# Kelicious/faster_rcnn

Hardware: AMD Instinct MI355X
Metric: images/sec end-to-end (RPN+det) ResNet-50 600x1000 (higher is better)
Workload: dtype f32

## Files before the change

faster_rcnn_amd/_lib.py:

```python
import ctypes
import os
from ctypes import c_char_p, c_double, c_int, c_size_t, c_void_p

HERE = os.path.dirname(os.path.abspath(__file__))
LIB_PATH = os.environ.get("FRCNN_LIB_PATH") or os.path.join(HERE, "libfrcnn_hip.so")


class FrcnnError(RuntimeError):
    pass


ABI_VERSION = 110
P = c_void_p
I = c_int
SIGNATURES = {
    "frcnn_last_error": (c_char_p, []),
    "frcnn_version": (I, []),
    "frcnn_device_count": (I, []),
    "frcnn_preprocess_u8": (I, [P, c_size_t, P, P, P]),
    "frcnn_resize_cubic_taps": (I, [I, I, P]),
    "frcnn_resize_cubic_u8": (I, [P, I, I, P, P, I, I, I, P, P]),
    "frcnn_anchors_image": (I, [I, I, P, I, I, P, P]),
    "frcnn_anchors_conv": (I, [I, I, P, I, P, P]),
    "frcnn_cross_ious_f32": (I, [P, I, P, I, P, P]),
# ... 58 lines not shown
    "frcnn_conv2d_fwd_ws_amax": (I, [P, P, P, P, P, P, P, P, P, P, c_size_t, P]),
    "frcnn_pack_conv_weights_dgrad": (I, [P, P, I, I, I, I, P, P]),
    "frcnn_conv2d_wgrad_workspace_bytes": (c_size_t, [P]),
    "frcnn_conv2d_wgrad": (I, [P, P, P, P, P, P, P, c_size_t, P]),
    "frcnn_conv2d_wgrad_batch_workspace_bytes": (c_size_t, [P, I]),
    "frcnn_conv2d_wgrad_batch": (I, [P, I, P, c_size_t, P]),
    "frcnn_refresh_packed": (I, [P, I, P]),
    "frcnn_colsum_batch": (I, [P, I, P]),
    "frcnn_pool2d_fwd": (I, [P, I, I, I, I, I, I, I, P, P]),
    "frcnn_pool2d_fwd_planes": (I, [P, I, I, I, I, I, I, I, P, P]),
    "frcnn_avgpool_pos_major": (I, [P, I, I, I, P, P]),
    "frcnn_softmax_rows": (I, [P, I, I, I, P, I, P]),
    "frcnn_dense_heads_split": (I, [P, I, I, I, I, P, P, P]),
    "frcnn_loss_rpn_cls": (I, [P, P, I, I, P, P, P]),
    "frcnn_loss_rpn_reg": (I, [P, P, I, I, P, P, P]),
    "frcnn_loss_workspace_bytes": (ctypes.c_size_t, []),
    "frcnn_loss_rpn_cls_ws": (I, [P, P, I, I, P, P, P, P]),
    "frcnn_loss_rpn_reg_ws": (I, [P, P, I, I, P, P, P, P]),
    "frcnn_loss_det_cls": (I, [P, P, I, I, P, P, I, P]),
    "frcnn_loss_det_reg": (I, [P, P, I, I, P, P, I, P]),
    "frcnn_relu_bwd_inplace": (I, [P, P, c_size_t, P]),
    "frcnn_avgpool_bwd_masked": (I, [P, P, I, I, I, P, P]),
    "frcnn_maxpool_bwd": (I, [P, P, P, I, I, I, I, I, P, P]),
    "frcnn_sgd_momentum": (I, [P, P, P, c_size_t, ctypes.c_float, ctypes.c_float, ctypes.c_float, ctypes.c_float, P]),
    "frcnn_adam": (I, [P, P, P, P, c_size_t, ctypes.c_float, ctypes.c_float, ctypes.c_float, ctypes.c_float, I, ctypes.c_float, ctypes.c_float, P]),
    "frcnn_sumsq_workspace_bytes": (c_size_t, []),
    "frcnn_sumsq": (I, [P, c_size_t, P, P, c_size_t, P]),
    "frcnn_fold_bias": (I, [P, P, P, P, I, P]),
    "frcnn_stem_bf16_packed_elems": (I, []),
    "frcnn_pack_stem_weights_bf16": (I, [P, P, P]),
    "frcnn_stem_bf16_fwd": (I, [P, I, I, I, P, P, P, P, P]),
    "frcnn_conv_packed_k_bf16": (I, [I, I, I]),
    "frcnn_pack_conv_weights_bf16": (I, [P, I, I, I, I, P, P]),
    "frcnn_conv2d_fwd_bf16": (I, [P, P, P, P, P, P, P, I, P]),
    "frcnn_conv2d_workspace_bytes_bf16": (c_size_t, [P]),
    "frcnn_conv2d_fwd_bf16_ws": (I, [P, P, P, P, P, P, P, I, P, c_size_t, P]),
    "frcnn_conv2d_fwd_bf16_masked": (I, [P, P, P, P, P, P, P, P, I, P, c_size_t, P]),
    "frcnn_refresh_packed_bf16": (I, [P, I, P]),
    "frcnn_conv2d_wgrad_bf16": (I, [P, P, P, P, P, P, P, c_size_t, P]),
    "frcnn_cast_bf16_to_f32": (I, [P, c_size_t, P, P]),
    "frcnn_relu_bwd_inplace_bf16": (I, [P, P, c_size_t, P]),
    "frcnn_avgpool_bwd_masked_bf16": (I, [P, P, I, I, I, P, P]),
    "frcnn_roi_crop_resize_bwd_bf16": (I, [P, I, I, I, P, I, I, P, P]),
    "frcnn_cast_f32_to_bf16": (I, [P, c_size_t, P, P]),
    "frcnn_avgpool_bf16_to_f32": (I, [P, I, I, I, P, P]),
    "frcnn_avgpool_bf16_to_f32_ex": (I, [P, I, I, I, I, P, P]),
    "frcnn_roi_crop_resize_fwd_bf16": (I, [P, I, I, I, P, I, I, P, P]),
    "frcnn_roi_crop_resize_fwd_bf16_ex": (I, [P, I, I, I, P, I, I, P, I, I, P, P]),
    "frcnn_roi_crop_resize_fwd_bf16_batch": (I, [P, I, I, I, I, P, I, I, P, I, I, P, P]),
    "frcnn_detections": (I, [P, P, I, P, P, I, I, c_double, c_double, c_double, c_double, P, P, P, P, P, P]),
    "frcnn_detections_dyn": (I, [P, P, I, I, P, P, I, I, c_double, c_double, P, P, P, P, P, P, P]),
    "frcnn_annotate_u8": (I, [P, I, I, P, P, P, P, I, P, P, I, I, P, P]),
    "frcnn_vgg_conv1_bf16_packed_elems": (I, []),
    "frcnn_pack_vgg_conv1_weights_bf16": (I, [P, P, P]),
    "frcnn_vgg_conv1_bf16_fwd": (I, [P, I, I, I, P, P, P, P]),
    "frcnn_pool2d_fwd_bf16": (I, [P, I, I, I, I, I, I, P, P]),
}

VGG_CANVAS_VERSION = 1
EXT_SIGNATURES = {
    "frcnn_vgg_canvas_version": (I, []),
    "frcnn_pool2d_fwd_extents": (I, [P, I, I, I, I, P, P, P]),
    "frcnn_pool2d_fwd_bf16_extents": (I, [P, I, I, I, I, P, P, P]),
    "frcnn_vgg_conv1_bf16_fwd_extents": (I, [P, I, I, I, P, P, P, P, P]),
}

ROI_RES_VERSION = 1
ROI_TAP_BYTES = 32
ROI_RES_SIGNATURES = {
    "frcnn_roi_res_version": (I, []),
    "frcnn_roi_tap_table": (I, [I, I, I, P, I, I, I, I, I, P, P]),
    "frcnn_conv2d_roi_res_available": (I, [P, I, I]),
    "frcnn_conv2d_fwd_h3_roi_res": (I, [P, P, P, P, P, P, P, P, P, P, P, P, ctypes.c_float, ctypes.c_float, P]),
}


POOL_EPILOGUE_VERSION = 1
POOL_EPILOGUE_SIGNATURES = {
    "frcnn_pool_epilogue_version": (I, []),
    "frcnn_conv2d_pool_available": (I, [P, I, I, I]),
    "frcnn_conv2d_fwd_h3_pool": (I, [P, P, P, P, P, P, P, P, P, P, I, P, P, P, P]),
}


class RoiRes(ctypes.Structure):
    _fields_ = [("map", c_void_p), ("taps", c_void_p), ("fill", c_void_p), ("map_rows", ctypes.c_int32), ("reserved", ctypes.c_int32)]


PNG_VERSION = 1
PNG_SIGNATURES = {
    "frcnn_png_version": (I, []),
    "frcnn_png_band_rows": (I, []),
    "frcnn_png_bound": (c_size_t, [I, I]),
    "frcnn_png_workspace_bytes": (c_size_t, [I, I]),
    "frcnn_png_encode_u8": (I, [P, I, I, I, P, c_size_t, P, P, P]),
}

PNG_HUFF_VERSION = 1
PNG_HUFF_SIGNATURES = {
    "frcnn_png_huff_version": (I, []),
    "frcnn_png_huff_band_rows": (I, []),
    "frcnn_png_huff_bound": (c_size_t, [I, I]),
    "frcnn_png_huff_workspace_bytes": (c_size_t, [I, I]),
    "frcnn_png_huff_encode_u8": (I, [P, I, I, I, P, c_size_t, P, P, P]),
}

JPEG_VERSION = 1
JPEG_SIGNATURES = {
    "frcnn_jpeg_version": (I, []),
    "frcnn_jpeg_restart_mcus": (I, []),
    "frcnn_jpeg_header_bytes": (c_size_t, []),
    "frcnn_jpeg_bound": (c_size_t, [I, I]),
    "frcnn_jpeg_workspace_bytes": (c_size_t, [I, I]),
    "frcnn_jpeg_encode_u8": (I, [P, I, I, I, I, P, c_size_t, P, P, P]),
}

JPEG_OPT_VERSION = 1
JPEG_OPT_SIGNATURES = {
    "frcnn_jpeg_opt_version": (I, []),
    "frcnn_jpeg_opt_restart_mcus": (I, [I]),
    "frcnn_jpeg_opt_bound": (c_size_t, [I, I, I]),
    "frcnn_jpeg_opt_workspace_bytes": (c_size_t, [I, I, I, I]),
    "frcnn_jpeg_opt_encode_u8": (I, [P, I, I, I, I, I, I, P, c_size_t, P, P, P]),
    "frcnn_jpeg_opt_build_tables": (I, [P, P, P]),
}
JPEG_OPT_SUBSAMPLINGS = (444, 420)
JPEG_OPT_HUFFMANS = {"standard": 0, "optimized": 1}


class JpegOptTable(ctypes.Structure):
    _fields_ = [("bits", ctypes.c_uint8 * 16), ("huffval", ctypes.c_uint8 * 256), ("count", ctypes.c_uint32)]


JPEG_DEC_VERSION = 1
JPEG_DEC_SIGNATURES = {
    "frcnn_jpeg_dec_version": (I, []),
    "frcnn_jpeg_dec_plan": (I, [P, c_size_t, P]),
    "frcnn_jpeg_dec_workspace_bytes": (c_size_t, [P]),
    "frcnn_jpeg_decode_u8": (I, [P, P, I, P, c_size_t, P, P, P]),
}
JPEG_DEC_BATCH_VERSION = 1
JPEG_DEC_BATCH_MAX = 64
JPEG_DEC_BATCH_SIGNATURES = {
    "frcnn_jpeg_dec_batch_version": (I, []),
    "frcnn_jpeg_dec_batch_layout": (c_size_t, [P, I, P]),
    "frcnn_jpeg_decode_batch_u8": (I, [P, P, I, P, c_size_t, I, P, c_size_t, P, P, c_size_t, P]),
}
E_UNSUPPORTED = -4
JPEG_DEC_BLOCKS, JPEG_DEC_ZIGZAG, JPEG_DEC_CODE, JPEG_DEC_TABLE = 1, 2, 4, 8


PNG_DEC_VERSION = 1
PNG_DEC_BATCH_MAX = 64
PNG_DEC_WINDOW_BYTES = 8192
PNG_DEC_MAX_STREAM = 1 << 24
PNG_DEC_SIGNATURES = {
    "frcnn_png_dec_version": (I, []),
    "frcnn_png_dec_plan": (I, [P, c_size_t, P]),
    "frcnn_png_dec_spans": (I, [P, c_size_t, P, P, c_size_t]),
    "frcnn_png_dec_workspace_bytes": (c_size_t, [P]),
    "frcnn_png_dec_batch_layout": (c_size_t, [P, I, P]),
    "frcnn_png_decode_batch_u8": (I, [P, P, I, P, c_size_t, I, P, c_size_t, P, P, c_size_t, P]),
}
PNG_DEC_CODE, PNG_DEC_BLOCK, PNG_DEC_OVERSUBSCRIBED, PNG_DEC_DISTANCE, PNG_DEC_OVERRUN, PNG_DEC_UNDERRUN, PNG_DEC_ADLER, PNG_DEC_FILTER = \
    1, 2, 4, 8, 16, 32, 64, 128

# ... 154 lines not shown
    "frcnn_track_trails_update": (I, [P, I, P, ctypes.c_longlong, I, I, P, P, I, I, I, I, P, P]),
    "frcnn_track_trails_draw_u8": (I, [P, I, I, P, I, I, I, P]),
}
TRACK_TRAILS = ((2, 64, 16), (1, 9, 3), 4095)

TRACK_LOOKBACK_VERSION = 1
TRACK_LOOKBACK_SIGNATURES = {
    "frcnn_track_lookback_version": (I, []),
    "frcnn_track_lookback_state_bytes": (c_size_t, [I, I, I, I, I, I]),
    "frcnn_track_lookback": (I, [P, P, ctypes.c_longlong, P, ctypes.c_longlong, I, P, I, I, I, I, I, I, I, I, P, ctypes.c_longlong, P,
                                 ctypes.c_longlong, P, P]),
}
TRACK_LOOKBACK = (1, 16, 8)
TRACK_LOOKBACK_MAX_BACK = 128
TRACK_LOOKBACK_HEADER = 32

TRACK_BACKTRACK_VERSION = 1
TRACK_BACKTRACK_SIGNATURES = {
    "frcnn_track_backtrack_version": (I, []),
    "frcnn_track_backtrack": (I, [P, P, ctypes.c_longlong, P, ctypes.c_longlong, I, P, I, I, I, I, I, I, I, I, I, P, ctypes.c_longlong, P,
                                  ctypes.c_longlong, P, P]),
}


class ConvDesc(ctypes.Structure):
    _fields_ = [(k, ctypes.c_int32) for k in (
        "n", "h", "w", "cin", "cout", "kh", "kw", "stride", "pad_top", "pad_left", "ho", "wo",
        "act", "ldy", "ldres", "tile", "layout")]


class PackJob(ctypes.Structure):
    _fields_ = [(k, c_void_p) for k in ("w_hwio", "packed", "packed_dgrad", "bias", "scale", "shift_const", "shift")] + \
               [(k, ctypes.c_int32) for k in ("kh", "kw", "cin", "cout")]


class WgradJob(ctypes.Structure):
    _fields_ = [("d", ConvDesc)] + [(k, c_void_p) for k in ("x", "g", "scale", "dw")] + [(k, ctypes.c_int32) for k in ("in_bf16", "reserved")]


class X6Job(ctypes.Structure):
    _fields_ = [("w_packed", c_void_p), ("planes_bf16", c_void_p), ("rows", ctypes.c_int32), ("kpad", ctypes.c_int32)]


H3_UNDER, H3_SATURATED, H3_NONFINITE = 1, 2, 4


class H3Planes(ctypes.Structure):
    _fields_ = [("planes", c_void_p), ("exponent", c_void_p), ("status", c_void_p)]


class ColsumJob(ctypes.Structure):
    _fields_ = [(k, c_void_p) for k in ("g", "scale", "out")] + [(k, ctypes.c_int32) for k in ("m", "cout", "g_is_bf16", "reserved")]


_lib = None


def load():
    global _lib
    if _lib is not None:
        return _lib
    if not os.path.exists(LIB_PATH):
        raise FrcnnError(
            f"{LIB_PATH} is missing: build it with `python -m faster_rcnn_amd.build` "
            "(hipcc --offload-arch=gfx950).  There is no CPU fallback.")
    import torch
    lib = ctypes.CDLL(LIB_PATH)
    for name, (res, args) in SIGNATURES.items():
        fn = getattr(lib, name)
        fn.restype = res
        fn.argtypes = args
    for name, (res, args) in EXT_SIGNATURES.items():
        fn = getattr(lib, name)
        fn.restype = res
        fn.argtypes = args
    for name, (res, args) in ROI_RES_SIGNATURES.items():
        fn = getattr(lib, name)
        fn.restype = res
        fn.argtypes = args
    for name, (res, args) in POOL_EPILOGUE_SIGNATURES.items():
        fn = getattr(lib, name)
        fn.restype = res
        fn.argtypes = args
    for name, (res, args) in PNG_SIGNATURES.items():
        fn = getattr(lib, name)
        fn.restype = res
        fn.argtypes = args
    for name, (res, args) in PNG_HUFF_SIGNATURES.items():
        fn = getattr(lib, name)
        fn.restype = res
        fn.argtypes = args
    for name, (res, args) in JPEG_SIGNATURES.items():
        fn = getattr(lib, name)
        fn.restype = res
        fn.argtypes = args
    for name, (res, args) in JPEG_OPT_SIGNATURES.items():
        fn = getattr(lib, name)
        fn.restype = res
        fn.argtypes = args
    for name, (res, args) in JPEG_DEC_SIGNATURES.items():
        fn = getattr(lib, name)
        fn.restype = res
        fn.argtypes = args
    for name, (res, args) in JPEG_DEC_BATCH_SIGNATURES.items():
        fn = getattr(lib, name)
        fn.restype = res
        fn.argtypes = args
    for name, (res, args) in PNG_DEC_SIGNATURES.items():
        fn = getattr(lib, name)
        fn.restype = res
        fn.argtypes = args
    for name, (res, args) in PNG_DEC_FULL_SIGNATURES.items():
        fn = getattr(lib, name)
        fn.restype = res
        fn.argtypes = args
    for name, (res, args) in JPEG_DEC_FULL_SIGNATURES.items():
        fn = getattr(lib, name)
        fn.restype = res
        fn.argtypes = args
    for name, (res, args) in Y4M_SIGNATURES.items():
        fn = getattr(lib, name)
        fn.restype = res
        fn.argtypes = args
    for name, (res, args) in REDACT_SIGNATURES.items():
        fn = getattr(lib, name)
        fn.restype = res
        fn.argtypes = args
    for name, (res, args) in TRACK_SIGNATURES.items():
        fn = getattr(lib, name)
        fn.restype = res
        fn.argtypes = args
    if lib.frcnn_track_version() != TRACK_VERSION:
        raise FrcnnError(f"{LIB_PATH} speaks revision {lib.frcnn_track_version()} of the tracking extension, this binding "
                         f"{TRACK_VERSION} (include/ext/frcnn_hip_track.h): rebuild with `python -m faster_rcnn_amd.build`")
    for name, (res, args) in TRACK_MOTION_SIGNATURES.items():
        fn = getattr(lib, name)
        fn.restype = res
        fn.argtypes = args
    if lib.frcnn_track_motion_version() != TRACK_MOTION_VERSION:
        raise FrcnnError(f"{LIB_PATH} speaks revision {lib.frcnn_track_motion_version()} of the tracker's motion extension, this binding "
                         f"{TRACK_MOTION_VERSION} (include/ext/frcnn_hip_track_motion.h): rebuild with `python -m faster_rcnn_amd.build`")
    for name, (res, args) in TRACK_LOOKBACK_SIGNATURES.items():
        fn = getattr(lib, name)
        fn.restype = res
        fn.argtypes = args
    if lib.frcnn_track_lookback_version() != TRACK_LOOKBACK_VERSION:
        raise FrcnnError(f"{LIB_PATH} speaks revision {lib.frcnn_track_lookback_version()} of the tracker's look-back extension, this binding "
                         f"{TRACK_LOOKBACK_VERSION} (include/ext/frcnn_hip_track_lookback.h): rebuild with `python -m faster_rcnn_amd.build`")
    for name, (res, args) in TRACK_BACKTRACK_SIGNATURES.items():
        fn = getattr(lib, name, None)
        if fn is None:
            raise FrcnnError(f"{LIB_PATH} has no {name} (include/ext/frcnn_hip_track_backtrack.h): rebuild with `python -m faster_rcnn_amd.build`")
        fn.restype = res
        fn.argtypes = args
    if lib.frcnn_track_backtrack_version() != TRACK_BACKTRACK_VERSION:
        raise FrcnnError(f"{LIB_PATH} speaks revision {lib.frcnn_track_backtrack_version()} of the tracker's back-track extension, this binding "
                         f"{TRACK_BACKTRACK_VERSION} (include/ext/frcnn_hip_track_backtrack.h): rebuild with `python -m faster_rcnn_amd.build`")
    for name, (res, args) in TRACK_INTERVAL_SIGNATURES.items():
        fn = getattr(lib, name)
        fn.restype = res
        fn.argtypes = args
    if lib.frcnn_track_interval_version() != TRACK_INTERVAL_VERSION:
        raise FrcnnError(f"{LIB_PATH} speaks revision {lib.frcnn_track_interval_version()} of the tracker's interval extension, this binding "
                         f"{TRACK_INTERVAL_VERSION} (include/ext/frcnn_hip_track_interval.h): rebuild with `python -m faster_rcnn_amd.build`")
    for name, (res, args) in TRACK_CUT_SIGNATURES.items():
        fn = getattr(lib, name, None)
# ... 76 lines not shown
```

faster_rcnn_amd/csrc/stem_h3.hip:

```cpp
#include "conv_f32_common.h"

namespace frcnn {

typedef _Float16 sf16x8 __attribute__((ext_vector_type(8)));

constexpr int SH_PH = 4, SH_PW = 16;
constexpr int SH_CH = 2 * SH_PH + 1, SH_CW = 2 * SH_PW + 1;
constexpr int SH_CM = SH_CH * SH_CW;
constexpr int SH_MT = (SH_CM + 31) / 32;
constexpr int SH_IH = 2 * SH_CH + 5, SH_IW = 2 * SH_CW + 5;
constexpr int SH_ROW = 216;
constexpr int SH_PROWS = SH_IH + 2;
constexpr int SH_K = 176, SH_WLD = 184;
constexpr int SH_CLD = 68;
constexpr int SH_NT = 512;
constexpr size_t SH_PATCH = (size_t)SH_PROWS * SH_ROW * 2, SH_FILT = (size_t)64 * SH_WLD * 2;
constexpr size_t SH_LDS = 2 * SH_PATCH + 2 * SH_FILT + (size_t)SH_CM * SH_CLD * 4;
constexpr int SH_HEADER = 16;

__host__ __device__ __forceinline__ int sh_exponent(float amax) {
    unsigned b;
    __builtin_memcpy(&b, &amax, 4);
    const int e = 141 - (int)((b >> 23) & 0xffu);
    return e > 100 ? 100 : (e < -100 ? -100 : e);
}
__host__ __device__ __forceinline__ float sh_pow2(int e) {
    const unsigned b = (unsigned)(e + 127) << 23;
    float f;
    __builtin_memcpy(&f, &b, 4);
    return f;
}

__global__ void __launch_bounds__(SH_NT) k_stem_h3(const float* __restrict__ x, const float* __restrict__ x_amax, const char* __restrict__ wp,
                                                   const float* __restrict__ scale, const float* __restrict__ shift, int H, int W, int Hp, int Wp,
                                                   float* __restrict__ out, float* __restrict__ y_amax) {
    extern __shared__ __attribute__((aligned(16))) char sh_smem[];
    _Float16* patch = reinterpret_cast<_Float16*>(sh_smem);
    _Float16* wl = reinterpret_cast<_Float16*>(sh_smem + 2 * SH_PATCH);
    float* ct = reinterpret_cast<float*>(sh_smem + 2 * SH_PATCH + 2 * SH_FILT);
    const int tid = threadIdx.x, lane = tid & 63, wave = tid >> 6, li = lane & 31, lh = lane >> 5;
    const int px0 = blockIdx.x * SH_PW, py0 = blockIdx.y * SH_PH, img = blockIdx.z;
    const int Ho = (H + 1) / 2, Wo = (W + 1) / 2;
    const int pad_t = max((Ho - 1) * 2 + 7 - H, 0) / 2, pad_l = max((Wo - 1) * 2 + 7 - W, 0) / 2;
    const int iy0 = 4 * py0 - pad_t, ix0 = 4 * px0 - pad_l;
    const float* xi = x + (size_t)img * H * W * 3;

    constexpr int NP = (SH_PROWS * SH_ROW + SH_NT - 1) / SH_NT;
    float pv[NP];
#pragma unroll
    for (int q = 0; q < NP; ++q) {
        const int idx = tid + q * SH_NT;
        const int row = idx / SH_ROW, col = idx - row * SH_ROW;
        const int gy = iy0 + row, gx = ix0 + col / 3;
        const bool ok = idx < SH_PROWS * SH_ROW && row < SH_IH && col < SH_IW * 3 && (unsigned)gy < (unsigned)H && (unsigned)gx < (unsigned)W;
        pv[q] = ok ? xi[(size_t)gy * W * 3 + (ix0 * 3 + col)] : 0.0f;
    }
    h3_fp16_saturate();
    const float x_max = amax_read(x_amax);
    const int eA = sh_exponent(x_max);
    const int eB = sh_exponent(*reinterpret_cast<const float*>(wp));
    const float sA = sh_pow2(eA);
    h3_check_record(x_amax, x_max);
    unsigned seen = 0u;
#pragma unroll
    for (int q = 0; q < NP; ++q) {
        const int idx = tid + q * SH_NT;
        if (idx < SH_PROWS * SH_ROW) {
            const float xs = pv[q] * sA;
            const _Float16 hi = (_Float16)xs;
            h3_see(seen, hi);
            patch[idx] = hi;
            patch[SH_PROWS * SH_ROW + idx] = (_Float16)((xs - (float)hi) * 2048.0f);
        }
    }
    h3_report(x_amax, seen);
    const _Float16* wsrc = reinterpret_cast<const _Float16*>(wp + SH_HEADER);
    for (int idx = tid; idx < 2 * 64 * (SH_K / 8); idx += SH_NT) {
        const int pl = idx / (64 * (SH_K / 8)), r = idx - pl * (64 * (SH_K / 8)), n = r / (SH_K / 8), c8 = r - n * (SH_K / 8);
        *reinterpret_cast<i32x4*>(wl + pl * 64 * SH_WLD + n * SH_WLD + c8 * 8) = *reinterpret_cast<const i32x4*>(wsrc + pl * 64 * SH_K + n * SH_K + c8 * 8);
    }
    __syncthreads();

    const float unscale_a = sh_pow2(-eA), unscale_b = sh_pow2(-eB);
    for (int u = wave; u < 2 * SH_MT; u += SH_NT / 64) {
        const int mt = u >> 1, ct_col = (u & 1) * 32;
        const int m = mt * 32 + li, mm = m < SH_CM ? m : 0;
        const int cy = mm / SH_CW, cx = mm - cy * SH_CW;
        const _Float16* arow = patch + (2 * cy) * SH_ROW + 6 * cx;
        const _Float16* brow = wl + (ct_col + li) * SH_WLD + lh * 8;
        f32x16 acc0, acc1;
#pragma unroll
        for (int e = 0; e < 16; ++e) { acc0[e] = 0.0f; acc1[e] = 0.0f; }
#pragma unroll
        for (int kt = 0; kt < SH_K / 16; ++kt) {
            const int g = 2 * kt + lh, r = g / 3, j0 = (g - 3 * r) * 8;
            const unsigned* ah = reinterpret_cast<const unsigned*>(arow + r * SH_ROW + j0);
            const unsigned* al = ah + SH_PROWS * SH_ROW / 2;
            const i32x4 avh = {(int)ah[0], (int)ah[1], (int)ah[2], (int)ah[3]}, avl = {(int)al[0], (int)al[1], (int)al[2], (int)al[3]};
            const sf16x8 fah = __builtin_bit_cast(sf16x8, avh), fal = __builtin_bit_cast(sf16x8, avl);
            const sf16x8 fbh = *reinterpret_cast<const sf16x8*>(brow + kt * 16);
            const sf16x8 fbl = *reinterpret_cast<const sf16x8*>(brow + 64 * SH_WLD + kt * 16);
            acc1 = __builtin_amdgcn_mfma_f32_32x32x16_f16(fal, fbh, acc1, 0, 0, 0);
            acc1 = __builtin_amdgcn_mfma_f32_32x32x16_f16(fah, fbl, acc1, 0, 0, 0);
            acc0 = __builtin_amdgcn_mfma_f32_32x32x16_f16(fah, fbh, acc0, 0, 0, 0);
        }
        const float sc = scale[ct_col + li], sh = shift[ct_col + li];
#pragma unroll
        for (int e = 0; e < 16; ++e) {
            const int row = mt * 32 + (e & 3) + 8 * (e >> 2) + 4 * lh;
            if (row < SH_CM) {
                const float conv = ((acc0[e] + acc1[e] * (1.0f / 2048.0f)) * unscale_a) * unscale_b;
                ct[row * SH_CLD + ct_col + li] = fmaxf(conv * sc + sh, 0.0f);
            }
        }
    }
    __syncthreads();

    float vmax = 0.0f;
    for (int item = tid; item < SH_PH * SH_PW * 16; item += SH_NT) {
        const int pix = item >> 4, c4 = item & 15;
        const int ppy = pix / SH_PW, ppx = pix - ppy * SH_PW;
        const int py = py0 + ppy, px = px0 + ppx;
        if (py < Hp && px < Wp) {
            f32x4 best = {0.0f, 0.0f, 0.0f, 0.0f};
#pragma unroll
            for (int dy = 0; dy < 3; ++dy)
#pragma unroll
                for (int dx = 0; dx < 3; ++dx) {
                    const f32x4 v = *reinterpret_cast<const f32x4*>(ct + ((2 * ppy + dy) * SH_CW + 2 * ppx + dx) * SH_CLD + c4 * 4);
#pragma unroll
                    for (int q = 0; q < 4; ++q) best[q] = fmaxf(best[q], v[q]);
                }
            *reinterpret_cast<f32x4*>(out + (((size_t)img * Hp + py) * Wp + px) * 64 + c4 * 4) = best;
            vmax = fmaxf(fmaxf(vmax, fmaxf(best[0], best[1])), fmaxf(best[2], best[3]));
        }
    }
    if (y_amax) amax_publish(y_amax, vmax);
}

__global__ void k_stem_h3_wmax(const float* w, unsigned* header) {
    float v = 0.0f;
    for (int i = blockIdx.x * blockDim.x + threadIdx.x; i < 7 * 7 * 3 * 64; i += gridDim.x * blockDim.x) v = fmaxf(v, fabsf(w[i]));
    v = wave_max(v);
    if ((threadIdx.x & 63) == 0 && v > 0.0f) atomicMax(header, __float_as_uint(v));
}

__global__ void k_pack_stem_h3(const float* w, char* packed) {
    const float s = sh_pow2(sh_exponent(*reinterpret_cast<const float*>(packed)));
    _Float16* out = reinterpret_cast<_Float16*>(packed + SH_HEADER);
    for (int i = blockIdx.x * blockDim.x + threadIdx.x; i < 64 * SH_K; i += gridDim.x * blockDim.x) {
        const int n = i / SH_K, k = i - n * SH_K, r = k / 24, j = k - r * 24, sx = j / 3, c = j - sx * 3;
        const float v = (r < 7 && j < 21) ? w[((r * 7 + sx) * 3 + c) * 64 + n] * s : 0.0f;
        const _Float16 hi = (_Float16)v;
        out[i] = hi;
        out[64 * SH_K + i] = (_Float16)((v - (float)hi) * 2048.0f);
    }
}

__global__ void k_stem_h3_zero_header(unsigned* header) { if (threadIdx.x < SH_HEADER / 4) header[threadIdx.x] = 0u; }

}

using namespace frcnn;

extern "C" {

size_t frcnn_stem_h3_packed_bytes(void) { return (size_t)SH_HEADER + (size_t)2 * 64 * SH_K * 2; }

int frcnn_pack_stem_weights_h3(const float* w_hwio, void* packed, void* stream) {
    if (!w_hwio || !packed) return fail(FRCNN_E_ARG, "pack_stem_weights_h3: null pointer");
    if (reinterpret_cast<uintptr_t>(packed) & 15) return fail(FRCNN_E_ARG, "pack_stem_weights_h3: 16-byte aligned buffer required");
    hipStream_t s = as_stream(stream);
    k_stem_h3_zero_header<<<1, 64, 0, s>>>(reinterpret_cast<unsigned*>(packed));
    k_stem_h3_wmax<<<37, 256, 0, s>>>(w_hwio, reinterpret_cast<unsigned*>(packed));
    k_pack_stem_h3<<<44, 256, 0, s>>>(w_hwio, reinterpret_cast<char*>(packed));
    return check_launch("pack_stem_weights_h3");
}

int frcnn_stem_h3_fwd(const float* x, const float* x_amax, int n, int h, int w, const void* w_packed, const float* scale, const float* shift,
                      float* out, float* y_amax, void* stream) {
    if (!x || !x_amax || !w_packed || !scale || !shift || !out) return fail(FRCNN_E_ARG, "stem_h3_fwd: null pointer (the image's magnitude record is required)");
    if (n <= 0 || h < 7 || w < 7) return fail(FRCNN_E_ARG, "stem_h3_fwd: bad shape");
    const int ho = (h + 1) / 2, wo = (w + 1) / 2, hp = (ho - 3) / 2 + 1, wp = (wo - 3) / 2 + 1;
    if (hp <= 0 || wp <= 0) return fail(FRCNN_E_ARG, "stem_h3_fwd: image too small for the 3x3 pool");
    if ((reinterpret_cast<uintptr_t>(w_packed) | reinterpret_cast<uintptr_t>(out)) & 15) return fail(FRCNN_E_ARG, "stem_h3_fwd: 16-byte aligned tensors");
    static std::atomic<uint64_t> lds_seen{0};
    if (int e = raise_lds_once(lds_seen, (const void*)k_stem_h3, SH_LDS, "stem_h3_fwd")) return e;
    const dim3 grid((wp + SH_PW - 1) / SH_PW, (hp + SH_PH - 1) / SH_PH, n);
    if (grid.y > 65535 || grid.z > 65535) return fail(FRCNN_E_ARG, "stem_h3_fwd: image too large");
    k_stem_h3<<<grid, SH_NT, SH_LDS, as_stream(stream)>>>(x, x_amax, reinterpret_cast<const char*>(w_packed), scale, shift, h, w, hp, wp, out, y_amax);
    return check_launch("stem_h3_fwd");
}

}
```

faster_rcnn_amd/ops.py:

```python
import ctypes
import dataclasses
import os

import numpy as np
import torch

from . import _lib
from . import y4m as _y4m

NMS_MAX_BOXES = 12288


_GPU_SEEN = False


def _require_gpu():
    global _GPU_SEEN
    if not _GPU_SEEN:
        if not torch.cuda.is_available():
            raise _lib.FrcnnError("no HIP device visible: the faster_rcnn_amd ops need an MI355X (no CPU fallback)")
        _GPU_SEEN = True


_RAW_STREAM = getattr(torch._C, "_cuda_getCurrentRawStream", None)
# ... 2168 lines not shown
    _lib.call("frcnn_cast_f32_to_bf16", _p(x.contiguous()), x.numel(), _p(out), _stream())
    return out


def avgpool_bf16(x, k, layout=0):
    _require_gpu()
    n, c = (x.shape[2] if layout else x.shape[0]), x.shape[3]
    out = torch.empty((n, c), dtype=torch.float32, device="cuda")
    _lib.call("frcnn_avgpool_bf16_to_f32_ex", _p(x.contiguous()), n, k, c, layout, _p(out), _stream())
    return out


def roi_crop_resize_bf16(feat, rois, pool, fill=None, relu=False, layout=0):
    _require_gpu()
    feat = feat.reshape(feat.shape[-3], feat.shape[-2], feat.shape[-1]).contiguous()
    rows, cols, C = feat.shape
    rois = rois.reshape(-1, 4).to(torch.float32).contiguous()
    n = rois.shape[0]
    out = torch.empty((pool, pool, n, C) if layout else (n, pool, pool, C), dtype=torch.bfloat16, device="cuda")
    _lib.call("frcnn_roi_crop_resize_fwd_bf16_ex", _p(feat), rows, cols, C, _p(rois), n, pool, _p(fill), 1 if relu else 0, layout, _p(out), _stream())
    return out


def roi_crop_resize_bf16_batch(feat, rois, n_per_img, pool, fill=None, relu=False, layout=0):
    _require_gpu()
    assert feat.dtype == torch.bfloat16 and feat.dim() == 4 and feat.is_contiguous()
    B, rows, cols, C = feat.shape
    rois = rois.reshape(-1, 4).to(torch.float32).contiguous()
    n = rois.shape[0]
    assert n == B * n_per_img
    out = torch.empty((pool, pool, n, C) if layout else (n, pool, pool, C), dtype=torch.bfloat16, device="cuda")
    _lib.call("frcnn_roi_crop_resize_fwd_bf16_batch", _p(feat), B, rows, cols, C, _p(rois), n_per_img, pool, _p(fill), 1 if relu else 0, layout, _p(out), _stream())
    return out


class PackedStemBf16:

    def __init__(self, w_hwio, scale, shift):
        _require_gpu()
        w = _dev(w_hwio, torch.float32)
        assert tuple(w.shape) == (7, 7, 3, 64), "the fused stem is conv1 of the ResNets: 7x7x3 -> 64"
        self.w = torch.empty(_lib.load().frcnn_stem_bf16_packed_elems(), dtype=torch.bfloat16, device="cuda")
        _lib.call("frcnn_pack_stem_weights_bf16", _p(w), _p(self.w), _stream())
        self.scale, self.shift = _dev(scale, torch.float32), _dev(shift, torch.float32)
        torch.cuda.current_stream().synchronize()


def stem_bf16(x, ps):
    _require_gpu()
    assert x.dtype == torch.float32 and x.is_contiguous() and x.dim() == 4 and x.shape[-1] == 3
    n, h, w, _ = x.shape
    ho, wo = (h + 1) // 2, (w + 1) // 2
    out = torch.empty((n, (ho - 3) // 2 + 1, (wo - 3) // 2 + 1, 64), dtype=torch.bfloat16, device="cuda")
    _lib.call("frcnn_stem_bf16_fwd", _p(x), n, h, w, _p(ps.w), _p(ps.scale), _p(ps.shift), _p(out), _stream())
    return out


class PackedStemH3:

    def __init__(self, w_hwio, scale, shift):
        _require_gpu()
        w = _dev(w_hwio, torch.float32)
        assert tuple(w.shape) == (7, 7, 3, 64), "the fused stem is conv1 of the ResNets: 7x7x3 -> 64"
        self.w = torch.empty(_lib.load().frcnn_stem_h3_packed_bytes(), dtype=torch.uint8, device="cuda")
        _lib.call("frcnn_pack_stem_weights_h3", _p(w), _p(self.w), _stream())
        self.scale, self.shift = _dev(scale, torch.float32), _dev(shift, torch.float32)
        torch.cuda.current_stream().synchronize()


def stem_h3(x, ps):
    _require_gpu()
    assert x.dtype == torch.float32 and x.is_contiguous() and x.dim() == 4 and x.shape[-1] == 3
    n, h, w, _ = x.shape
    ho, wo = (h + 1) // 2, (w + 1) // 2
    out = torch.empty((n, (ho - 3) // 2 + 1, (wo - 3) // 2 + 1, 64), dtype=torch.float32, device="cuda")
    ya, xa = _amax_new(), amax_of(x)
    args = (_p(x), _p(xa), n, h, w, _p(ps.w), _p(ps.scale), _p(ps.shift), _p(out), _p(ya))
    _lib.call("frcnn_stem_h3_fwd", *args, _stream())
    out._amax = ya
    _record_launch(lambda: "k_stem_h3", (n * ho * wo, 64, 147, 2), "frcnn_stem_h3_fwd", args, (x, ps, out, ya, xa))
    return out


class PackedVggConv1Bf16:

    def __init__(self, w_hwio, bias):
        _require_gpu()
        w = _dev(w_hwio, torch.float32)
        assert tuple(w.shape) == (3, 3, 3, 64), "the conv1 kernel is block1_conv1 of VGG16: 3x3x3 -> 64"
        self.w = torch.empty(_lib.load().frcnn_vgg_conv1_bf16_packed_elems(), dtype=torch.bfloat16, device="cuda")
        _lib.call("frcnn_pack_vgg_conv1_weights_bf16", _p(w), _p(self.w), _stream())
        self.bias = _dev(bias, torch.float32)
        torch.cuda.current_stream().synchronize()


def vgg_conv1_bf16(x, packed):
    _require_gpu()
    assert x.dtype == torch.float32 and x.is_contiguous() and x.dim() == 4 and x.shape[-1] == 3
    n, h, w, _ = x.shape
    out = torch.empty((n, h, w, 64), dtype=torch.bfloat16, device="cuda")
    args = (_p(x), n, h, w, _p(packed.w), _p(packed.bias), _p(out))
    _lib.call("frcnn_vgg_conv1_bf16_fwd", *args, _stream())
    _record_launch(lambda: "k_vgg_conv1_bf16", (n * h * w, 64, 27, 1), "frcnn_vgg_conv1_bf16_fwd", args, (x, packed, out))
    return out


def pool2d_bf16(x, k, stride):
    _require_gpu()
    assert x.dtype == torch.bfloat16 and x.is_contiguous() and x.dim() == 4
    n, h, w, c = x.shape
    out = torch.empty((n, valid_out(h, k, stride), valid_out(w, k, stride), c), dtype=torch.bfloat16, device="cuda")
    args = (_p(x), n, h, w, c, k, stride, _p(out))
    _lib.call("frcnn_pool2d_fwd_bf16", *args, _stream())
    _record_launch(lambda: "k_pool2_bf16", (out.numel() // c, c, k * k, 1), "frcnn_pool2d_fwd_bf16", args, (x, out))
    return out


def vgg_conv1_bf16_extents(x, packed, true_hw):
    _require_gpu()
    assert x.dtype == torch.float32 and x.is_contiguous() and x.dim() == 4 and x.shape[-1] == 3
    assert true_hw.dtype == torch.int32 and true_hw.is_cuda and true_hw.numel() >= 2 * x.shape[0]
    n, h, w, _ = x.shape
    out = torch.empty((n, h, w, 64), dtype=torch.bfloat16, device="cuda")
    args = (_p(x), n, h, w, _p(packed.w), _p(packed.bias), _p(true_hw), _p(out))
    _lib.call("frcnn_vgg_conv1_bf16_fwd_extents", *args, _stream())
    _record_launch(lambda: "k_vgg_conv1_bf16", (n * h * w, 64, 27, 1), "frcnn_vgg_conv1_bf16_fwd_extents", args, (x, packed, out, true_hw))
    return out


def pool2d_bf16_extents(x, true_hw):
    _require_gpu()
    assert x.dtype == torch.bfloat16 and x.is_contiguous() and x.dim() == 4
    assert true_hw.dtype == torch.int32 and true_hw.is_cuda and true_hw.numel() >= 2 * x.shape[0]
    n, h, w, c = (int(v) for v in x.shape)
    out = torch.empty((n, h // 2, w // 2, c), dtype=torch.bfloat16, device="cuda")
    args = (_p(x), n, h, w, c, _p(true_hw), _p(out))
    _lib.call("frcnn_pool2d_fwd_bf16_extents", *args, _stream())
    _record_launch(lambda: "k_pool2_extents", (out.numel() // c, c, 4, 1), "frcnn_pool2d_fwd_bf16_extents", args, (x, out, true_hw))
    return out
```

Baseline: 560.9.

## Add persistent stem kernel with register-held filters and double-buffered patch prefetch

Adds a persistent form of the fused stem conv+BN+ReLU+maxpool kernel. A grid of at most one workgroup per compute unit walks the patches in a strided loop. Each wave keeps its filter fragments in registers instead of reloading them from LDS per patch. The next patch's global loads are issued before the MFMA work on the current patch, and the patch buffer is double-buffered in LDS. This is meant to amortise filter loading and block launch overhead and to hide input-load latency, at the cost of higher register pressure and only one 512-thread workgroup per CU. The persistent form is the default and can be turned off with an environment variable.

```diff
diff --git a/faster_rcnn_amd/_lib.py b/faster_rcnn_amd/_lib.py
--- a/faster_rcnn_amd/_lib.py
+++ b/faster_rcnn_amd/_lib.py
@@ -164,6 +164,15 @@
     "frcnn_conv2d_fwd_h3_pool": (I, [P, P, P, P, P, P, P, P, P, P, I, P, P, P, P]),
 }
 
+STEM_H3_PERSISTENT_VERSION = 1
+STEM_H3_FORM_PATCH, STEM_H3_FORM_PERSISTENT = 0, 1
+STEM_H3_PERSISTENT_SIGNATURES = {
+    "frcnn_stem_h3_persistent_version": (I, []),
+    "frcnn_stem_h3_default_form": (I, []),
+    "frcnn_stem_h3_workgroups": (I, [I, I, I, I, I]),
+    "frcnn_stem_h3_fwd_form": (I, [P, P, I, I, I, P, P, P, P, P, I, I, P]),
+}
+
 
 class RoiRes(ctypes.Structure):
     _fields_ = [("map", c_void_p), ("taps", c_void_p), ("fill", c_void_p), ("map_rows", ctypes.c_int32), ("reserved", ctypes.c_int32)]
@@ -484,6 +493,15 @@
         fn = getattr(lib, name)
         fn.restype = res
         fn.argtypes = args
+    for name, (res, args) in STEM_H3_PERSISTENT_SIGNATURES.items():
+        fn = getattr(lib, name, None)
+        if fn is None:
+            raise FrcnnError(f"{LIB_PATH} has no {name} (include/ext/frcnn_hip_stem_h3_persistent.h): rebuild with `python -m faster_rcnn_amd.build`")
+        fn.restype = res
+        fn.argtypes = args
+    if lib.frcnn_stem_h3_persistent_version() != STEM_H3_PERSISTENT_VERSION:
+        raise FrcnnError(f"{LIB_PATH} speaks revision {lib.frcnn_stem_h3_persistent_version()} of the stem's launch-form extension, this binding "
+                         f"{STEM_H3_PERSISTENT_VERSION} (include/ext/frcnn_hip_stem_h3_persistent.h): rebuild with `python -m faster_rcnn_amd.build`")
     for name, (res, args) in PNG_SIGNATURES.items():
         fn = getattr(lib, name)
         fn.restype = res
diff --git a/faster_rcnn_amd/csrc/stem_h3.hip b/faster_rcnn_amd/csrc/stem_h3.hip
--- a/faster_rcnn_amd/csrc/stem_h3.hip
+++ b/faster_rcnn_amd/csrc/stem_h3.hip
@@ -1,10 +1,13 @@
 #include "conv_f32_common.h"
+#include "stem_h3_walk.h"
+#include "../../include/ext/frcnn_hip_stem_h3_persistent.h"
 
 namespace frcnn {
 
 typedef _Float16 sf16x8 __attribute__((ext_vector_type(8)));
 
 constexpr int SH_PH = 4, SH_PW = 16;
+static_assert(SH_PH == SH_WALK_PH && SH_PW == SH_WALK_PW, "stem_h3_walk.h walks these patches");
 constexpr int SH_CH = 2 * SH_PH + 1, SH_CW = 2 * SH_PW + 1;
 constexpr int SH_CM = SH_CH * SH_CW;
 constexpr int SH_MT = (SH_CM + 31) / 32;
@@ -31,9 +34,9 @@
     return f;
 }
 
-__global__ void __launch_bounds__(SH_NT) k_stem_h3(const float* __restrict__ x, const float* __restrict__ x_amax, const char* __restrict__ wp,
-                                                   const float* __restrict__ scale, const float* __restrict__ shift, int H, int W, int Hp, int Wp,
-                                                   float* __restrict__ out, float* __restrict__ y_amax) {
+__global__ void __launch_bounds__(SH_NT) k_stem_h3_patch(const float* __restrict__ x, const float* __restrict__ x_amax, const char* __restrict__ wp,
+                                                         const float* __restrict__ scale, const float* __restrict__ shift, int H, int W, int Hp, int Wp,
+                                                         float* __restrict__ out, float* __restrict__ y_amax) {
     extern __shared__ __attribute__((aligned(16))) char sh_smem[];
     _Float16* patch = reinterpret_cast<_Float16*>(sh_smem);
     _Float16* wl = reinterpret_cast<_Float16*>(sh_smem + 2 * SH_PATCH);
@@ -138,6 +141,149 @@
     if (y_amax) amax_publish(y_amax, vmax);
 }
 
+constexpr size_t SH_LDS_P = 4 * SH_PATCH + (size_t)SH_CM * SH_CLD * 4;
+
+__global__ void __launch_bounds__(SH_NT) k_stem_h3(const float* __restrict__ x, const float* __restrict__ x_amax, const char* __restrict__ wp,
+                                                   const float* __restrict__ scale, const float* __restrict__ shift, int H, int W, ShWalk walk,
+                                                   float* __restrict__ out, float* __restrict__ y_amax) {
+    extern __shared__ __attribute__((aligned(16))) char sh_smem[];
+    _Float16* pbuf = reinterpret_cast<_Float16*>(sh_smem);
+    float* ct = reinterpret_cast<float*>(sh_smem + 4 * SH_PATCH);
+    constexpr int PLANE = SH_PROWS * SH_ROW;
+    const int tid = threadIdx.x, lane = tid & 63, wave = tid >> 6, li = lane & 31, lh = lane >> 5;
+    const int total = (int)walk.patches, G = gridDim.x, Hp = walk.hp, Wp = walk.wp;
+    const int Ho = (H + 1) / 2, Wo = (W + 1) / 2;
+    const int pad_t = max((Ho - 1) * 2 + 7 - H, 0) / 2, pad_l = max((Wo - 1) * 2 + 7 - W, 0) / 2;
+
+    constexpr int NP = (PLANE + SH_NT - 1) / SH_NT;
+    unsigned pk[NP];
+#pragma unroll
+    for (int q = 0; q < NP; ++q) {
+        const int idx = tid + q * SH_NT;
+        const int row = idx / SH_ROW, col = idx - row * SH_ROW;
+        const bool in = idx < PLANE && row < SH_IH && col < SH_IW * 3;
+        pk[q] = (unsigned)row | (unsigned)(col / 3) << 8 | (unsigned)col << 16 | (in ? 0x80000000u : 0u);
+    }
+    float pv[NP];
+    unsigned pin = 0u;
+    auto load_patch = [&](int p) {
+        int img, py0, px0;
+        sh_walk_origin(walk, p, &img, &py0, &px0);
+        const int iy0 = 4 * py0 - pad_t, ix0 = 4 * px0 - pad_l;
+        const float* xi = x + (size_t)img * H * W * 3;
+        pin = 0u;
+#pragma unroll
+        for (int q = 0; q < NP; ++q) {
+            const int gy = iy0 + (int)(pk[q] & 0xffu), gx = ix0 + (int)((pk[q] >> 8) & 0xffu), col = (int)((pk[q] >> 16) & 0xffu);
+            const bool ok = (int)pk[q] < 0 && (unsigned)gy < (unsigned)H && (unsigned)gx < (unsigned)W;
+            pv[q] = xi[ok ? (size_t)gy * W * 3 + (ix0 * 3 + col) : (size_t)0];
+            pin |= ok ? 1u << q : 0u;
+        }
+    };
+    int p = blockIdx.x;
+    load_patch(p);
+    const int ct_col = (wave & 1) * 32, wq = wave >> 1;
+    const _Float16* bsrc = reinterpret_cast<const _Float16*>(wp + SH_HEADER) + (ct_col + li) * SH_K + lh * 8;
+    sf16x8 fbh[SH_K / 16], fbl[SH_K / 16];
+#pragma unroll
+    for (int kt = 0; kt < SH_K / 16; ++kt) {
+        fbh[kt] = *reinterpret_cast<const sf16x8*>(bsrc + kt * 16);
+        fbl[kt] = *reinterpret_cast<const sf16x8*>(bsrc + 64 * SH_K + kt * 16);
+    }
+    const float sc = scale[ct_col + li], sh = shift[ct_col + li];
+    h3_fp16_saturate();
+    const float x_max = amax_read(x_amax);
+    const int eA = sh_exponent(x_max);
+    const int eB = sh_exponent(*reinterpret_cast<const float*>(wp));
+    const float sA = sh_pow2(eA);
+    const float unscale_a = sh_pow2(-eA), unscale_b = sh_pow2(-eB);
+    h3_check_record(x_amax, x_max);
+    unsigned seen = 0u;
+    auto store_patch = [&](_Float16* dst) {
+#pragma unroll
+        for (int q = 0; q < NP; ++q) {
+            const int idx = tid + q * SH_NT;
+            if (idx < PLANE) {
+                const float xs = ((pin >> q) & 1u ? pv[q] : 0.0f) * sA;
+                const _Float16 hi = (_Float16)xs;
+                h3_see(seen, hi);
+                dst[idx] = hi;
+                dst[PLANE + idx] = (_Float16)((xs - (float)hi) * 2048.0f);
+            }
+        }
+    };
+    store_patch(pbuf);
+    __syncthreads();
+
+    float vmax = 0.0f;
+    for (int cur = 0; p < total; p += G, cur ^= 1) {
+        const _Float16* patch = pbuf + cur * 2 * PLANE;
+        const bool more = p + G < total;
+        if (more) load_patch(p + G);
+        for (int mt = wq; mt < SH_MT; mt += SH_NT / 128) {
+            const int m = mt * 32 + li, mm = m < SH_CM ? m : 0;
+            const int cy = mm / SH_CW, cx = mm - cy * SH_CW;
+            const _Float16* arow = patch + (2 * cy) * SH_ROW + 6 * cx;
+            f32x16 acc0, acc1;
+#pragma unroll
+            for (int e = 0; e < 16; ++e) { acc0[e] = 0.0f; acc1[e] = 0.0f; }
+            auto read_a = [&](int kt, i32x4& avh, i32x4& avl) {
+                const int g = 2 * kt + lh, r = g / 3, j0 = (g - 3 * r) * 8;
+                const unsigned* ah = reinterpret_cast<const unsigned*>(arow + r * SH_ROW + j0);
+                const unsigned* al = ah + PLANE / 2;
+                avh = i32x4{(int)ah[0], (int)ah[1], (int)ah[2], (int)ah[3]};
+                avl = i32x4{(int)al[0], (int)al[1], (int)al[2], (int)al[3]};
+            };
+            i32x4 nvh, nvl;
+            read_a(0, nvh, nvl);
+#pragma unroll
+            for (int kt = 0; kt < SH_K / 16; ++kt) {
+                const sf16x8 fah = __builtin_bit_cast(sf16x8, nvh), fal = __builtin_bit_cast(sf16x8, nvl);
+                if (kt + 1 < SH_K / 16) read_a(kt + 1, nvh, nvl);
+                __builtin_amdgcn_sched_barrier(0);
+                acc1 = __builtin_amdgcn_mfma_f32_32x32x16_f16(fal, fbh[kt], acc1, 0, 0, 0);
+                acc1 = __builtin_amdgcn_mfma_f32_32x32x16_f16(fah, fbl[kt], acc1, 0, 0, 0);
+                acc0 = __builtin_amdgcn_mfma_f32_32x32x16_f16(fah, fbh[kt], acc0, 0, 0, 0);
+                __builtin_amdgcn_sched_barrier(0);
+            }
+#pragma unroll
+            for (int e = 0; e < 16; ++e) {
+                const int row = mt * 32 + (e & 3) + 8 * (e >> 2) + 4 * lh;
+                if (row < SH_CM) {
+                    const float conv = ((acc0[e] + acc1[e] * (1.0f / 2048.0f)) * unscale_a) * unscale_b;
+                    ct[row * SH_CLD + ct_col + li] = fmaxf(conv * sc + sh, 0.0f);
+                }
+            }
+        }
+        if (more) store_patch(pbuf + (cur ^ 1) * 2 * PLANE);
+        __syncthreads();
+
+        int img, py0, px0;
+        sh_walk_origin(walk, p, &img, &py0, &px0);
+        for (int item = tid; item < SH_PH * SH_PW * 16; item += SH_NT) {
+            const int pix = item >> 4, c4 = item & 15;
+            const int ppy = pix / SH_PW, ppx = pix - ppy * SH_PW;
+            const int py = py0 + ppy, px = px0 + ppx;
+            if (py < Hp && px < Wp) {
+                f32x4 best = {0.0f, 0.0f, 0.0f, 0.0f};
+#pragma unroll
+                for (int dy = 0; dy < 3; ++dy)
+#pragma unroll
+                    for (int dx = 0; dx < 3; ++dx) {
+                        const f32x4 v = *reinterpret_cast<const f32x4*>(ct + ((2 * ppy + dy) * SH_CW + 2 * ppx + dx) * SH_CLD + c4 * 4);
+#pragma unroll
+                        for (int q = 0; q < 4; ++q) best[q] = fmaxf(best[q], v[q]);
+                    }
+                *reinterpret_cast<f32x4*>(out + (((size_t)img * Hp + py) * Wp + px) * 64 + c4 * 4) = best;
+                vmax = fmaxf(fmaxf(vmax, fmaxf(best[0], best[1])), fmaxf(best[2], best[3]));
+            }
+        }
+        __syncthreads();
+    }
+    h3_report(x_amax, seen);
+    if (y_amax) amax_publish(y_amax, vmax);
+}
+
 __global__ void k_stem_h3_wmax(const float* w, unsigned* header) {
     float v = 0.0f;
     for (int i = blockIdx.x * blockDim.x + threadIdx.x; i < 7 * 7 * 3 * 64; i += gridDim.x * blockDim.x) v = fmaxf(v, fabsf(w[i]));
@@ -163,6 +309,8 @@
 
 using namespace frcnn;
 
+static const bool g_stem_h3_persistent = !(getenv("FRCNN_STEM_H3_PERSISTENT") && atoi(getenv("FRCNN_STEM_H3_PERSISTENT")) == 0);
+
 extern "C" {
 
 size_t frcnn_stem_h3_packed_bytes(void) { return (size_t)SH_HEADER + (size_t)2 * 64 * SH_K * 2; }
@@ -177,19 +325,61 @@
     return check_launch("pack_stem_weights_h3");
 }
 
+static int stem_h3_compute_units(int* cus) {
+    static std::atomic<int> cached[64];
+    int dev = 0;
+    if (hipGetDevice(&dev) != hipSuccess) return fail(FRCNN_E_HIP, "stem_h3_fwd: no current HIP device");
+    int v = cached[dev & 63].load(std::memory_order_acquire);
+    if (v <= 0) {
+        if (hipDeviceGetAttribute(&v, hipDeviceAttributeMultiprocessorCount, dev) != hipSuccess || v <= 0)
+            return fail(FRCNN_E_HIP, "stem_h3_fwd: cannot read the compute-unit count of device %d", dev);
+        cached[dev & 63].store(v, std::memory_order_release);
+    }
+    *cus = v;
+    return FRCNN_OK;
+}
+
+int frcnn_stem_h3_persistent_version(void) { return FRCNN_STEM_H3_PERSISTENT_VERSION; }
+
+int frcnn_stem_h3_default_form(void) { return g_stem_h3_persistent ? FRCNN_STEM_H3_FORM_PERSISTENT : FRCNN_STEM_H3_FORM_PATCH; }
+
+int frcnn_stem_h3_workgroups(int n, int h, int w, int compute_units, int max_workgroups) {
+    if (n <= 0 || h < 7 || w < 7 || compute_units <= 0) return fail(FRCNN_E_ARG, "stem_h3_workgroups: bad shape or compute-unit count");
+    const ShWalk walk = sh_walk(n, h, w);
+    if (walk.patches <= 0 || walk.patches + compute_units > 0x7fffffffll) return fail(FRCNN_E_ARG, "stem_h3_workgroups: image too small or too large");
+    return sh_walk_grid(walk.patches, compute_units, max_workgroups);
+}
+
+int frcnn_stem_h3_fwd_form(const float* x, const float* x_amax, int n, int h, int w, const void* w_packed, const float* scale, const float* shift,
+                           float* out, float* y_amax, int form, int max_workgroups, void* stream) {
+    if (!x || !x_amax || !w_packed || !scale || !shift || !out) return fail(FRCNN_E_ARG, "stem_h3_fwd: null pointer (the image's magnitude record is required)");
+    if (n <= 0 || h < 7 || w < 7) return fail(FRCNN_E_ARG, "stem_h3_fwd: bad shape");
+    if (form != FRCNN_STEM_H3_FORM_PATCH && form != FRCNN_STEM_H3_FORM_PERSISTENT) return fail(FRCNN_E_ARG, "stem_h3_fwd: unknown form %d", form);
+    const ShWalk walk = sh_walk(n, h, w);
+    if (walk.patches <= 0) return fail(FRCNN_E_ARG, "stem_h3_fwd: image too small for the 3x3 pool");
+    if ((reinterpret_cast<uintptr_t>(w_packed) | reinterpret_cast<uintptr_t>(out)) & 15) return fail(FRCNN_E_ARG, "stem_h3_fwd: 16-byte aligned tensors");
+    if (walk.py > 65535 || n > 65535) return fail(FRCNN_E_ARG, "stem_h3_fwd: image too large");
+    const char* wpk = reinterpret_cast<const char*>(w_packed);
+    if (form == FRCNN_STEM_H3_FORM_PATCH) {
+        static std::atomic<uint64_t> lds_seen{0};
+        if (int e = raise_lds_once(lds_seen, (const void*)k_stem_h3_patch, SH_LDS, "stem_h3_fwd")) return e;
+        const dim3 grid(walk.px, walk.py, n);
+        k_stem_h3_patch<<<grid, SH_NT, SH_LDS, as_stream(stream)>>>(x, x_amax, wpk, scale, shift, h, w, walk.hp, walk.wp, out, y_amax);
+        return check_launch("stem_h3_fwd");
+    }
+    int cus = 0;
+    if (int e = stem_h3_compute_units(&cus)) return e;
+    if (walk.patches + cus > 0x7fffffffll) return fail(FRCNN_E_ARG, "stem_h3_fwd: image too large");
+    static std::atomic<uint64_t> lds_seen_p{0};
+    if (int e = raise_lds_once(lds_seen_p, (const void*)k_stem_h3, SH_LDS_P, "stem_h3_fwd")) return e;
+    const int G = sh_walk_grid(walk.patches, cus, max_workgroups);
+    k_stem_h3<<<G, SH_NT, SH_LDS_P, as_stream(stream)>>>(x, x_amax, wpk, scale, shift, h, w, walk, out, y_amax);
+    return check_launch("stem_h3_fwd");
+}
+
 int frcnn_stem_h3_fwd(const float* x, const float* x_amax, int n, int h, int w, const void* w_packed, const float* scale, const float* shift,
                       float* out, float* y_amax, void* stream) {
-    if (!x || !x_amax || !w_packed || !scale || !shift || !out) return fail(FRCNN_E_ARG, "stem_h3_fwd: null pointer (the image's magnitude record is required)");
-    if (n <= 0 || h < 7 || w < 7) return fail(FRCNN_E_ARG, "stem_h3_fwd: bad shape");
-    const int ho = (h + 1) / 2, wo = (w + 1) / 2, hp = (ho - 3) / 2 + 1, wp = (wo - 3) / 2 + 1;
-    if (hp <= 0 || wp <= 0) return fail(FRCNN_E_ARG, "stem_h3_fwd: image too small for the 3x3 pool");
-    if ((reinterpret_cast<uintptr_t>(w_packed) | reinterpret_cast<uintptr_t>(out)) & 15) return fail(FRCNN_E_ARG, "stem_h3_fwd: 16-byte aligned tensors");
-    static std::atomic<uint64_t> lds_seen{0};
-    if (int e = raise_lds_once(lds_seen, (const void*)k_stem_h3, SH_LDS, "stem_h3_fwd")) return e;
-    const dim3 grid((wp + SH_PW - 1) / SH_PW, (hp + SH_PH - 1) / SH_PH, n);
-    if (grid.y > 65535 || grid.z > 65535) return fail(FRCNN_E_ARG, "stem_h3_fwd: image too large");
-    k_stem_h3<<<grid, SH_NT, SH_LDS, as_stream(stream)>>>(x, x_amax, reinterpret_cast<const char*>(w_packed), scale, shift, h, w, hp, wp, out, y_amax);
-    return check_launch("stem_h3_fwd");
-}
-
-}
+    return frcnn_stem_h3_fwd_form(x, x_amax, n, h, w, w_packed, scale, shift, out, y_amax, frcnn_stem_h3_default_form(), 0, stream);
+}
+
+}
diff --git a/faster_rcnn_amd/csrc/stem_h3_walk.h b/faster_rcnn_amd/csrc/stem_h3_walk.h
--- /dev/null
+++ b/faster_rcnn_amd/csrc/stem_h3_walk.h
@@ -0,0 +1,45 @@
+#pragma once
+
+#if defined(__HIPCC__) || defined(__CUDACC__)
+#define SH_WALK_FN __host__ __device__ inline
+#else
+#define SH_WALK_FN inline
+#endif
+
+namespace frcnn {
+
+constexpr int SH_WALK_PH = 4, SH_WALK_PW = 16;
+
+struct ShWalk {
+    int hp, wp;
+    int py, px;
+    long long patches;
+};
+
+SH_WALK_FN ShWalk sh_walk(int n, int h, int w) {
+    ShWalk k;
+    const int ho = (h + 1) / 2, wo = (w + 1) / 2;
+    k.hp = ho >= 3 ? (ho - 3) / 2 + 1 : 0;
+    k.wp = wo >= 3 ? (wo - 3) / 2 + 1 : 0;
+    k.py = (k.hp + SH_WALK_PH - 1) / SH_WALK_PH;
+    k.px = (k.wp + SH_WALK_PW - 1) / SH_WALK_PW;
+    k.patches = n > 0 ? (long long)n * k.py * k.px : 0;
+    return k;
+}
+
+SH_WALK_FN int sh_walk_grid(long long patches, int compute_units, int cap) {
+    long long g = patches < compute_units ? patches : compute_units;
+    if (cap > 0 && g > cap) g = cap;
+    return g < 0 ? 0 : (int)g;
+}
+
+SH_WALK_FN void sh_walk_origin(const ShWalk& k, long long p, int* img, int* py0, int* px0) {
+    const int per = k.py * k.px;
+    const int i = (int)(p / per), r = (int)(p - (long long)i * per);
+    const int by = r / k.px;
+    *img = i;
+    *py0 = by * SH_WALK_PH;
+    *px0 = (r - by * k.px) * SH_WALK_PW;
+}
+
+}
diff --git a/faster_rcnn_amd/ops.py b/faster_rcnn_amd/ops.py
--- a/faster_rcnn_amd/ops.py
+++ b/faster_rcnn_amd/ops.py
@@ -2274,6 +2274,22 @@
     return out
 
 
+def stem_h3_form(x, ps, form, max_workgroups=0, out=None):
+    _require_gpu()
+    assert x.dtype == torch.float32 and x.is_contiguous() and x.dim() == 4 and x.shape[-1] == 3
+    n, h, w, _ = x.shape
+    ho, wo = (h + 1) // 2, (w + 1) // 2
+    shape = (n, (ho - 3) // 2 + 1, (wo - 3) // 2 + 1, 64)
+    if out is None:
+        out = torch.empty(shape, dtype=torch.float32, device="cuda")
+    assert tuple(out.shape) == shape and out.dtype == torch.float32 and out.is_contiguous()
+    ya, xa = _amax_new(), amax_of(x)
+    _lib.call("frcnn_stem_h3_fwd_form", _p(x), _p(xa), n, h, w, _p(ps.w), _p(ps.scale), _p(ps.shift), _p(out), _p(ya), form, max_workgroups,
+              _stream())
+    out._amax = ya
+    return out, ya, xa
+
+
 class PackedVggConv1Bf16:
 
     def __init__(self, w_hwio, bias):
diff --git a/include/ext/frcnn_hip_stem_h3_persistent.h b/include/ext/frcnn_hip_stem_h3_persistent.h
--- /dev/null
+++ b/include/ext/frcnn_hip_stem_h3_persistent.h
@@ -0,0 +1,24 @@
+#ifndef FRCNN_HIP_STEM_H3_PERSISTENT_H
+#define FRCNN_HIP_STEM_H3_PERSISTENT_H
+#include <stdint.h>
+#include "../frcnn_hip.h"
+#ifdef __cplusplus
+extern "C" {
+#endif
+
+#define FRCNN_STEM_H3_PERSISTENT_VERSION 1
+int frcnn_stem_h3_persistent_version(void);
+
+#define FRCNN_STEM_H3_FORM_PATCH 0
+#define FRCNN_STEM_H3_FORM_PERSISTENT 1
+int frcnn_stem_h3_default_form(void);
+
+int frcnn_stem_h3_workgroups(int n, int h, int w, int compute_units, int max_workgroups);
+
+int frcnn_stem_h3_fwd_form(const float* x, const float* x_amax, int n, int h, int w, const void* w_packed, const float* scale,
+                           const float* shift, float* out, float* y_amax, int form, int max_workgroups, void* stream);
+
+#ifdef __cplusplus
+}
+#endif
+#endif
```

New measurement: 563.2 (median of 6 runs). No clear change (+0.4%).
